# wnmusic/simpleFE

Hardware: AMD Instinct MI355X
Metric: complex-float32 MS/s through 256-tap blkconv FIR; % of HBM roofline (higher is better)
Workload: dtype f32

## Files before the change

### simplefe_amd/build.py

```python
import glob
import json
import os
import subprocess
import sys

HERE = os.path.dirname(os.path.abspath(__file__))
CSRC = os.path.join(HERE, "csrc")
LIB = os.path.join(HERE, "libsfe_dsp.so")
LIB_DIAG = os.path.join(HERE, "libsfe_dsp_diag.so")
ARCH = "gfx950"
EXACT_SOURCES = ("polyphase.hip", "util.hip", "chan.hip", "combine.hip", "ddc.hip", "psd.hip", "corr.hip", "iir.hip", "beam.hip",
                 "cov.hip", "mvdr.hip", "eig.hip", "burst.hip", "vit.hip", "mod.hip")
TICKET_SOURCES = ("fir_fft.hip", "poly_fft.hip")
HOST_SOURCES = ("api.hip", "api_plans.hip", "api_fir.hip", "api_rs.hip", "api_pipe.hip", "api_chan.hip", "api_combine.hip", "api_ddc.hip",
                "api_psd.hip", "api_corr.hip", "api_iir.hip", "api_beam.hip", "api_cov.hip", "api_mvdr.hip", "api_eig.hip", "api_burst.hip", "api_vit.hip", "api_mod.hip", "group.hip", "host.h", "block.h",
                "beam_view.h", "vit_code.h")


def sources(diag=False):
    return sorted(glob.glob(os.path.join(CSRC, "*.hip"))) + (sorted(glob.glob(os.path.join(CSRC, "diag", "*.hip"))) if diag else [])


def _deps():
    return sources(diag=True) + glob.glob(os.path.join(CSRC, "*.h")) + glob.glob(os.path.join(CSRC, "diag", "*.inc")) + glob.glob(
        os.path.join(os.path.dirname(HERE), "include", "*.h"))


KERNEL_FILES = {"fir": ("fir_fft.hip", "fft16.h", "common.h"), "resample": ("poly_fft.hip", "fft16.h", "common.h"),
                "decimate": ("polyphase.hip", "common.h"), "chan": ("chan.hip", "fft16.h", "common.h"),
                "combine": ("combine.hip", "fft16.h", "common.h"), "ddc": ("ddc.hip", "common.h"),
                "psd": ("psd.hip", "fft16.h", "common.h"), "corr": ("corr.hip", "fft16.h", "common.h"),
                "iir": ("iir.hip", "iir.h", "common.h"), "beam": ("beam.hip", "beam.h", "common.h"),
                "cov": ("cov.hip", "cov.h", "common.h"), "mvdr": ("mvdr.hip", "mvdr.h", "beam.h", "common.h"),
                "eig": ("eig.hip", "eig.h", "common.h"), "burst": ("burst.hip", "burst.h", "eig.h", "common.h"),
                "vit": ("vit.hip", "vit.h", "burst.h", "eig.h", "common.h"),
                "mod": ("mod.hip", "mod.h", "vit.h", "burst.h", "eig.h", "common.h")}


def csrc_hash(kind=None):
    import hashlib
    import re
    h = hashlib.sha256()
    paths = sorted(glob.glob(os.path.join(CSRC, "*.hip")) + glob.glob(os.path.join(CSRC, "*.h")))
    if kind is not None:
        paths = [p for p in paths if os.path.basename(p) in KERNEL_FILES[kind]]
    for p in paths:
        if os.path.basename(p) in HOST_SOURCES:
            continue
        h.update(os.path.basename(p).encode() + b"\0")
        depth, skip_at = 0, None
        for line in open(p, errors="replace"):
            code = re.sub(r"\s+", " ", re.sub(r"//.*$", "", line)).strip()
            if code.startswith("#if"):
                depth += 1
                if skip_at is None and re.match(r"#ifdef SFE_DIAG\b", code):
                    skip_at = depth
                    continue
            elif code.startswith("#else") and skip_at == depth:
                skip_at = -depth
                continue
            elif code.startswith("#endif"):
# ... 139 lines not shown
```

### simplefe_amd/csrc/api_fir.hip

```cpp
#include "host.h"

namespace sfe {


Fir *as_fir(void *h) { return as_handle<Fir>(h, "FIR"); }

static int fir_build_tables(const Fir *f, const float *taps, int parts, int ovl, FirTables &t)
{
    const int N = FFT_N;
    std::vector<double> c(N / 2), sn(N / 2);
    for (int m = 0; m < N / 2; m++) {
        c[m] = cos(-2.0 * M_PI * m / N);
        sn[m] = sin(-2.0 * M_PI * m / N);
    }
    auto fft = [&](std::vector<double> &re, std::vector<double> &im) {
        for (int i = 1, j = 0; i < N; i++) {
            int bit = N >> 1;
            for (; j & bit; bit >>= 1) j ^= bit;
            j ^= bit;
            if (i < j) {
                std::swap(re[i], re[j]);
                std::swap(im[i], im[j]);
            }
        }
// ... 15 lines not shown
    std::vector<v2f> hs((size_t)n_sets * parts * 16 * 256), tw1(7 * 256), tw2(7 * 16);
    std::vector<double> hr(N), hi(N);
    for (int set = 0; set < n_sets; set++) {
    const float *tp = taps + (size_t)set * f->n_taps * (f->taps_complex ? 2 : 1);
    for (int p = 0; p < parts; p++) {
        const int first = parts == 1 ? 0 : p * ovl;
        const int count = parts == 1 ? f->n_taps : (f->n_taps - first < ovl ? f->n_taps - first : ovl);
        for (int n = 0; n < N; n++) {
            hr[n] = n < count ? (f->taps_complex ? tp[2 * (first + n)] : tp[first + n]) / (double)N : 0.0;
            hi[n] = n < count && f->taps_complex ? tp[2 * (first + n) + 1] / (double)N : 0.0;
        }
        fft(hr, hi);
        for (int t = 0; t < 256; t++)
            for (int k0 = 0; k0 < 16; k0++) {
                const int bin = (t >> 4) + 16 * (t & 15) + 256 * k0;
                hs[(((size_t)set * parts + p) * 16 + k0) * 256 + t] = (v2f){(float)hr[bin], (float)hi[bin]};
            }
    }
    }
    for (int k = 1; k < 4; k++)
        for (int t = 0; t < 256; t++) {
            const double a = -2.0 * M_PI * (double)(t * k) / 4096.0;
            tw1[k * 256 + t] = (v2f){(float)cos(a), (float)sin(a)};
            tw1[(k + 3) * 256 + t] = (v2f){(float)cos(4.0 * a), (float)sin(4.0 * a)};
        }
    for (int k = 1; k < 4; k++)
        for (int n0 = 0; n0 < 16; n0++) {
            const double a = -2.0 * M_PI * (double)(n0 * k) / 256.0;
            tw2[k * 16 + n0] = (v2f){(float)cos(a), (float)sin(a)};
            tw2[(k + 3) * 16 + n0] = (v2f){(float)cos(4.0 * a), (float)sin(4.0 * a)};
        }
    int rc;
    if ((rc = t.hs.upload(hs)) != SFE_OK || (rc = t.tw1.upload(tw1)) != SFE_OK || (rc = t.tw2.upload(tw2)) != SFE_OK) return rc;
    return t.ticket.alloc_zero(FIR_TICKET_GROUPS_MAX * 128 / sizeof(unsigned));
}

constexpr int FIR_MAX_PARTS = 1024;
static bool fir_choose_partition(int n_taps, int *ovl, int *parts)
{
    const int need = n_taps > 1 ? n_taps - 1 : 1;
    double best = 1e300;
    *parts = 0;
    const int hl1 = ((need + 255) / 256) * 256;
    if (hl1 < FFT_N) {
        best = 1.0 / (FFT_N - hl1);
        *ovl = hl1;
        *parts = 1;
    }
    for (int o = 256; o < FFT_N; o += 256) {
        const int P = (n_taps + o - 1) / o;
        if (P < 2 || P > FIR_MAX_PARTS) continue;
        const double cost = (P + 0.25 * (P - 1)) / (FFT_N - o);
        if (cost < best) {
            best = cost;
            *ovl = o;
            *parts = P;
        }
    }
    return *parts > 0;
}

bool stream_is_capturing(hipStream_t s)
{
    hipStreamCaptureStatus cap = hipStreamCaptureStatusNone;
    if (hipStreamIsCapturing(s, &cap) != hipSuccess) {
        (void)hipGetLastError();
        return false;
// ... 73 lines not shown
        if (v == 0) best_ms = med * FIR_CAL_MARGIN;
        else if (med < best_ms) {
            best_ms = med;
            best = v;
        }
    }
    f->cal_runs++;
    {
        std::lock_guard<std::mutex> lk(g_fir_var_mutex);
        g_fir_var_cache[fir_var_key(f, a)] = best;
    }
    *chosen = best;
    return SFE_OK;
}

static void fir_fill_args(const Fir *f, FirFftArgs &a, const void *d_in, void *d_out, size_t n, size_t in_stride,
                          size_t out_stride)
{
    a.in = d_in;
    a.out = d_out;
    a.hist = f->hist.cur();
    a.tw1 = f->tab.tw1;
    a.tw2 = f->tab.tw2;
    a.n = (long long)n;
    a.in_stride = (long long)in_stride;
    a.out_stride = (long long)out_stride;
    a.hl = f->ovl;
    a.advance = FFT_N - f->ovl;
    a.hist_len = f->hl;
    a.nblk = ((long long)n + a.advance - 1) / a.advance;
    a.ticket = f->tab.ticket;
    a.total = 0;
    a.tgroups = 0;
    a.hs_stride = f->per_channel ? (long long)f->parts * 16 * 256 : 0;
    a.variant = FIR_VAR_AUTO;
    a.hs = f->tab.hs;
    a.shift = 0;
    a.hist_out = nullptr;
}

static int fir_carry_state(Fir *f, const void *d_in, size_t n, size_t in_stride, bool fused, bool capturing, hipStream_t s)
{
    const int width = f->data_complex ? 2 : 1;
    if (capturing) {
        f->captured = true;
        return launch_history_update(d_in, (long long)n, (long long)in_stride, f->hist.cur(), f->hist.cur(), f->hl,
                                     width, f->n_channels, s, f->in_u8);
    }
    if (!fused) {
        int rc = launch_history_update(d_in, (long long)n, (long long)in_stride, f->hist.cur(), f->hist.next(),
                                       f->hl, width, f->n_channels, s, f->in_u8);
        if (rc != SFE_OK) return rc;
    }
    return f->hist.carry(f->captured, s);
}

int fir_run(Fir *f, const void *d_in, void *d_out, size_t n, size_t in_stride,
                   size_t out_stride, hipStream_t s)
{
    if (n == 0) return SFE_OK;
    f->started = true;
    int algo = f->algo;
    if (algo == SFE_FIR_ALGO_AUTO) algo = f->fft_ok ? SFE_FIR_ALGO_FFT : SFE_FIR_ALGO_DIRECT;
    int rc;
    bool hist_fused = false;
    const bool capturing = stream_is_capturing(s);
// ... 416 lines not shown
    int best = FIR_VAR_REG;
    int rc = fir_calibrate(f, a, s, &best);
    if (rc == SFE_OK && chosen) *chosen = best;
    return rc;
}

int sfe_dsp_fir_forget_calibrations(void)
{
    std::lock_guard<std::mutex> lk(g_fir_var_mutex);
    g_fir_var_cache.clear();
    return SFE_OK;
}

int sfe_dsp_fir_set_zero_copy_max(sfe_fir_t h, size_t max_samples)
{
    Fir *f = as_fir(h);
    if (!f) return SFE_EINVAL;
    if (f->stage.h) {
        set_error("fir_set_zero_copy_max: set it before the first sfe_dsp_fir_process_host call");
        return SFE_ESTATE;
    }
    f->zc_max = max_samples;
    return SFE_OK;
}

int sfe_dsp_fir_reset(sfe_fir_t h)
{
    Fir *f = as_fir(h);
    if (!f) return SFE_EINVAL;
    SFE_ON_DEVICE(f->device);
    SFE_HIP(hipDeviceSynchronize());
    const int rc = f->hist.zero();
    if (rc != SFE_OK) return rc;
    if (f->tab.ticket) SFE_HIP(hipMemset(f->tab.ticket, 0, FIR_TICKET_GROUPS_MAX * 128));
    f->started = false;
    return SFE_OK;
}

int sfe_dsp_fir_destroy(sfe_fir_t h)
{
    Fir *f = as_fir(h);
    if (!f) return SFE_OK;
    if (f->piped) {
        set_error("fir_destroy: a pipe still borrows this handle (sfe_dsp_pipe_destroy first)");
        return SFE_ESTATE;
    }
    return destroy_handle(f);
}

}
```

### simplefe_amd/csrc/common.h

```cpp
#pragma once
#include <hip/hip_runtime.h>
#include <stddef.h>
#include <stdint.h>

#include "../../include/sfe_dsp.h"

typedef float v2f __attribute__((ext_vector_type(2)));
typedef float v4f __attribute__((ext_vector_type(4)));

namespace sfe {

__device__ __forceinline__ void lds_barrier()
{
#if defined(__HIP_DEVICE_COMPILE__)
    asm volatile("s_waitcnt lgkmcnt(0)" ::: "memory");
    __builtin_amdgcn_s_barrier();
    asm volatile("" ::: "memory");
#endif
}

void set_error(const char *fmt, ...);
int hip_fail(hipError_t e, const char *what);
int device_cu_count();

// ... 13 lines not shown
};

#define SFE_HIP(call)                                         \
    do {                                                      \
        hipError_t e__ = (call);                              \
        if (e__ != hipSuccess) return ::sfe::hip_fail(e__, #call); \
    } while (0)

constexpr int FFT_N = 4096;
constexpr int FFT_ROWS = 16;
constexpr int LDS_K2_STRIDE = 272;
constexpr int LDS_K1_STRIDE = 17;
constexpr int WP_PITCH = 144;
constexpr int WP_REGION = 8 * WP_PITCH;

struct FirFftArgs {
    const void *in;
    void       *out;
    const void *hist;
    void       *hist_out;
    const v2f  *hs;
    const v2f  *tw1;
    const v2f  *tw2;
    long long   n;
    long long   in_stride, out_stride;
    int         hl;
    int         advance;
    int         hist_len;
    int         shift;
    long long   nblk;
    unsigned   *ticket;
    unsigned    total;
    unsigned    tgroups;
    unsigned    ch_groups;
    long long   hs_stride;
    unsigned    tqs;
    unsigned    halo_keep;
    int         variant;
};
enum { FIR_VAR_AUTO = -1, FIR_VAR_REG = 0, FIR_VAR_DMA = 1, FIR_VAR_WP = 2, FIR_VAR_COUNT = 3 };
bool fir_fft_has_variants(const FirFftArgs &a, int in_complex, int out_complex, int in_u8, int out_tx10, int n_channels, int accumulate);
constexpr int FIR_TICKET_GROUPS = 8;
constexpr int FIR_TICKET_GROUPS_MAX = 64;
int launch_fir_fft(const FirFftArgs &a, int in_complex, int out_complex, int in_u8, int out_tx10, int n_channels,
                   hipStream_t s, int accumulate = 0);

struct PolyArgs {
    const void *in;
    void       *out;
    const void *hist;
    const float *taps;
    long long   n_in, in_stride, out_stride;
    int         hl;
    int         U, plen;
    long long   pos0;
    int         step;
    long long   n_out;
    const long long *sched_pos;
    const float     *sched_mu;
};
int launch_poly_int(const PolyArgs &a, int data_complex, int taps_complex, int exact,
                    int n_channels, hipStream_t s);

struct PolyTiledPlan {
    int    SP = 0, UP = 0, Lp = 0, e_max = 0;
    float *d_G = nullptr;
    float *d_Gt = nullptr;
    int    gt_pitch = 8;
};
struct PolyTiledArgs {
    const void *in;
    void       *out;
    const void *hist;
    void       *hist_out = nullptr;
    unsigned    tiles = 0;
    unsigned    win = 0;
// ... 117 lines not shown
```

### simplefe_amd/csrc/diag/fir_fft_diag.inc

```
template <int WAVES>
__global__ __launch_bounds__(256, WAVES) void fir_copy_pattern_kernel(FirFftArgs a)
{
    const unsigned t = threadIdx.x;
    const char *in_c = static_cast<const char *>(a.in) + (size_t)blockIdx.y * a.in_stride * 8;
    char *out_c = static_cast<char *>(a.out) + (size_t)blockIdx.y * a.out_stride * 8;
    const int row0 = a.hl >> 8;
    for (long long blk = blockIdx.x; blk < a.nblk; blk += gridDim.x) {
        const long long base = blk * a.advance - a.hl;
        if (base < 0 || base + FFT_N > a.n) continue;
        v2f v[16];
#pragma unroll
        for (int r = 0; r < 16; r++) v[r] = load_sample<true>(in_c + (base + 256 * r) * 8, t);
#pragma unroll
        for (int r = 0; r < 16; r++)
            if (r >= row0) reinterpret_cast<v2f *>(out_c + (base + 256 * r) * 8)[t] = v[r];
    }
}


template <int WAVES>
__global__ __launch_bounds__(256, WAVES) void fir_copy_pattern16_kernel(FirFftArgs a)
{
    const unsigned t = threadIdx.x;
    const char *in_c = static_cast<const char *>(a.in) + (size_t)blockIdx.y * a.in_stride * 8;
    char *out_c = static_cast<char *>(a.out) + (size_t)blockIdx.y * a.out_stride * 8;
    const int row0 = a.hl >> 8;
    const unsigned half = t >> 7, col2 = t & 127;
    for (long long blk = blockIdx.x; blk < a.nblk; blk += gridDim.x) {
        const long long base = blk * a.advance - a.hl;
        if (base < 0 || base + FFT_N > a.n) continue;
        v4f v[8];
#pragma unroll
        for (int j = 0; j < 8; j++)
            v[j] = reinterpret_cast<const v4f *>(in_c + (base + 256 * (2 * j)) * 8)[col2 + 128 * half];
#pragma unroll
        for (int j = 0; j < 8; j++)
            if (2 * j + (int)half >= row0)
                reinterpret_cast<v4f *>(out_c + (base + 256 * (2 * j)) * 8)[col2 + 128 * half] = v[j];
    }
}

#define FIR_TRACE_WGS 163840
__device__ unsigned long long g_fir_trace[5 * FIR_TRACE_WGS];
__device__ unsigned long long g_fir_tdone[FIR_TRACE_WGS];
__device__ unsigned long long g_fir_tclk[FIR_TRACE_WGS];
__device__ int g_fir_gate;
__device__ int g_fir_order;

template <int WAVES, bool TICKET, bool BAR = false, bool TRACE = false>
__global__ __launch_bounds__(256, WAVES) void fir_copy_pattern_nt_kernel(FirFftArgs a)
{
    __shared__ unsigned s_next;
    const unsigned t = threadIdx.x;
    const unsigned long long t_start = TRACE ? wall_clock64() : 0ull;
    const int gate = TRACE ? g_fir_gate : 0;
    const int order = TRACE ? g_fir_order : 0;
    unsigned n_done = 0;
    const unsigned wg_lin = blockIdx.x + blockIdx.y * gridDim.x;
    auto leave = [&]() {
        if (TRACE && t == 0 && wg_lin < FIR_TRACE_WGS) {
            unsigned long long *r = g_fir_trace + 5ull * wg_lin;
            r[0] = t_start; r[1] = wall_clock64(); r[2] = n_done;
            r[3] = __builtin_amdgcn_s_getreg(20 | (3 << 11));
            r[4] = __builtin_amdgcn_s_getreg(4 | (31 << 11));
        }
    };
    const int row0 = a.hl >> 8;
    const unsigned nblk32 = (unsigned)a.nblk;
    const unsigned tg = a.tgroups, grp = blockIdx.x % tg;
    unsigned *const my_ticket = a.ticket + 32u * grp;
    const unsigned last_draw = (a.total > grp ? (a.total - grp + tg - 1u) / tg : 0u) + (gridDim.x - grp + tg - 1u) / tg - 1u;
    auto draw = [&]() -> unsigned {
        const unsigned c = __hip_atomic_fetch_add(my_ticket, 1u, __ATOMIC_RELAXED, __HIP_MEMORY_SCOPE_AGENT);
        if (c == last_draw) __hip_atomic_store(my_ticket, 0u, __ATOMIC_RELAXED, __HIP_MEMORY_SCOPE_AGENT);
        const unsigned long long k = (unsigned long long)c * tg + grp;
        return k < a.total ? (unsigned)k : 0xFFFFFFFFu;
// ... 203 lines not shown
```

### simplefe_amd/csrc/diag/fir_fft_launch_diag.inc

```
    if (ev && in_complex && out_complex && !in_u8 && !out_tx10) {
#define SFE_NEW(DM, DG, WPV) SFE_K(true, true, false, false, false, DM, DG, false, WPV)
#define SFE_NEW_DG(DM, WPV) do { if (diag == 1) SFE_NEW(DM, 1, WPV); else if (diag == 2) SFE_NEW(DM, 2, WPV); \
                                else if (diag == 3) SFE_NEW(DM, 3, WPV); else SFE_NEW(DM, 0, WPV); } while (0)
        bool done = true;
        const bool traced = (ev[0] == 'e' || ev[0] == 'E') && (getenv("SFE_FIR_TRACE") || getenv("SFE_FIR_ORDER") || getenv("SFE_FIR_GATE"));
        if (traced) {
            const int order = getenv("SFE_FIR_ORDER") ? atoi(getenv("SFE_FIR_ORDER")) : 0;
            SFE_HIP(hipMemcpyToSymbolAsync(HIP_SYMBOL(g_fir_order), &order, sizeof order, 0, hipMemcpyHostToDevice, s));
            const int gate = getenv("SFE_FIR_GATE") ? atoi(getenv("SFE_FIR_GATE")) : 0;
            SFE_HIP(hipMemcpyToSymbolAsync(HIP_SYMBOL(g_fir_gate), &gate, sizeof gate, 0, hipMemcpyHostToDevice, s));
        }
        if (ev[0] == 'c') hipLaunchKernelGGL((fir_copy_pattern_kernel<4>), grid2, block, 0, s, a);
        else if (ev[0] == 'd') hipLaunchKernelGGL((fir_copy_pattern16_kernel<4>), grid2, block, 0, s, a);
        else if (ev[0] == 'e' && traced) hipLaunchKernelGGL((fir_copy_pattern_nt_kernel<4, false, false, true>), grid2, block, 0, s, a);
        else if (ev[0] == 'E' && traced) hipLaunchKernelGGL((fir_copy_pattern_nt_kernel<4, true, false, true>), grid, block, 0, s, a);
        else if (ev[0] == 'e') hipLaunchKernelGGL((fir_copy_pattern_nt_kernel<4, false>), grid2, block, 0, s, a);
        else if (ev[0] == 'E') hipLaunchKernelGGL((fir_copy_pattern_nt_kernel<4, true>), grid, block, 0, s, a);
        else if (ev[0] == 'b') hipLaunchKernelGGL((fir_copy_pattern_nt_kernel<4, false, true>), grid2, block, 0, s, a);
        else if (ev[0] == 'g') hipLaunchKernelGGL((fir_copy_pattern_dma_kernel<4, true>), grid2, block, 0, s, a);
        else if (ev[0] == 'G') hipLaunchKernelGGL((fir_copy_pattern_dma_kernel<4, false>), grid2, block, 0, s, a);
        else if (ev[0] == 'q' || ev[0] == 'Q') {
            const int delay = getenv("SFE_FIR_DELAY") ? atoi(getenv("SFE_FIR_DELAY")) : 0;
            SFE_HIP(hipMemcpyToSymbolAsync(HIP_SYMBOL(g_fir_delay), &delay, sizeof delay, 0, hipMemcpyHostToDevice, s));
            if (ev[0] == 'q') hipLaunchKernelGGL((fir_copy_pattern_dma2_kernel<2, true>), grid2, block, 0, s, a);
            else hipLaunchKernelGGL((fir_copy_pattern_dma2_kernel<4, false>), grid2, block, 0, s, a);
        }
        else if (ev[0] == 'p') hipLaunchKernelGGL((fir_copy_pattern_pipe_kernel<4>), grid2, block, 0, s, a);
        else if (ev[0] == 'T') SFE_NEW_DG(false, false);
        else if (ev[0] == 'X') SFE_NEW_DG(true, false);
        else if (ev[0] == 'W') SFE_NEW_DG(true, true);
        else if (ev[0] == 'y') SFE_NEW(true, 8, false);
        else if (ev[0] == 'u') SFE_NEW(false, 8, false);
        else if (ev[0] == 'L') SFE_NEW(false, 16, false);
        else if (ev[0] == 'M') SFE_NEW(false, 32, false);
        else if (ev[0] == 'N') SFE_NEW(false, 48, false);
        else if (ev[0] == 'l') SFE_NEW(true, 16, false);
        else if (ev[0] == 'n') SFE_NEW(true, 48, false);
        else if (ev[0] == 'x') SFE_NEW(true, 4, false);
        else if (ev[0] == 't') SFE_NEW(false, 4, false);
        else if (ev[0] == 'w') SFE_NEW(true, 4, true);
        else done = false;
#undef SFE_NEW
#undef SFE_NEW_DG
        if (done) {
            SFE_HIP(hipGetLastError());
            if (const char *tp = getenv("SFE_FIR_TRACE")) {
                if (traced) {
                    const size_t nwg = (ev[0] == 'E' ? (size_t)grid.x : (size_t)grid2.x * grid2.y);
                    const size_t cnt = 5 * (nwg < FIR_TRACE_WGS ? nwg : FIR_TRACE_WGS);
                    unsigned long long *h = (unsigned long long *)malloc(cnt * 8);
                    SFE_HIP(hipStreamSynchronize(s));
                    SFE_HIP(hipMemcpyFromSymbol(h, HIP_SYMBOL(g_fir_trace), cnt * 8));
                    if (FILE *f = fopen(tp, "wb")) { fwrite(h, 8, cnt, f); fclose(f); }
                    free(h);
                    const size_t nt = a.total < FIR_TRACE_WGS ? a.total : FIR_TRACE_WGS;
                    h = (unsigned long long *)malloc(nt * 8);
                    SFE_HIP(hipMemcpyFromSymbol(h, HIP_SYMBOL(g_fir_tdone), nt * 8));
                    char tp2[512];
                    snprintf(tp2, sizeof tp2, "%s.done", tp);
                    if (FILE *f = fopen(tp2, "wb")) { fwrite(h, 8, nt, f); fclose(f); }
                    SFE_HIP(hipMemcpyFromSymbol(h, HIP_SYMBOL(g_fir_tclk), nt * 8));
                    snprintf(tp2, sizeof tp2, "%s.clk", tp);
                    if (FILE *f = fopen(tp2, "wb")) { fwrite(h, 8, nt, f); fclose(f); }
                    free(h);
                }
            }
            return SFE_OK;
        }
    }
```

### simplefe_amd/csrc/fir_fft.hip

```cpp
#include <stdint.h>
#include <stdlib.h>

#include "common.h"
#include "fft16.h"

namespace sfe {
namespace {

template <bool IN_C, bool IN_U8 = false>
__device__ __forceinline__ v2f load_sample(const void *p, unsigned lane)
{
    if constexpr (IN_U8) {
        if constexpr (IN_C) {
            const unsigned w = __builtin_nontemporal_load(reinterpret_cast<const unsigned short *>(p) + lane);
            return (v2f){u8_to_f32(w & 0xFFu), u8_to_f32(w >> 8)};
        } else {
            return (v2f){u8_to_f32(__builtin_nontemporal_load(reinterpret_cast<const unsigned char *>(p) + lane)), 0.0f};
        }
    }
    if constexpr (IN_C) return __builtin_nontemporal_load(reinterpret_cast<const v2f *>(p) + lane);
    else return (v2f){__builtin_nontemporal_load(reinterpret_cast<const float *>(p) + lane), 0.0f};
}

template <int K>
__device__ __forceinline__ unsigned quad_lane(unsigned v)
{
    return (unsigned)__builtin_amdgcn_update_dpp(0, (int)v, K | (K << 2) | (K << 4) | (K << 6), 0xF, 0xF, true);
}
__device__ __forceinline__ unsigned quad_odd(unsigned v)
{
    return (unsigned)__builtin_amdgcn_update_dpp(0, (int)v, 1 | (1 << 2) | (3 << 4) | (3 << 6), 0xF, 0xF, true);
}

__device__ __forceinline__ void store_group(unsigned char *d, unsigned u0, unsigned u1, unsigned u2, unsigned u3)
{
    const unsigned w = ((u0 >> 8) | ((u1 >> 8) << 2) | ((u2 >> 8) << 4) | ((u3 >> 8) << 6)) | ((u0 & 0xFFu) << 8) |
                       ((u1 & 0xFFu) << 16) | ((u2 & 0xFFu) << 24);
    __builtin_memcpy(d, &w, 4);
    d[4] = (unsigned char)u3;
}

#ifdef SFE_DIAG
__device__ unsigned long long g_fir_clk[4];
#define SFE_FIR_STAMP(i)                                                                   \
    do {                                                                                   \
        if (blockIdx.x == 0 && blockIdx.y == 0 && threadIdx.x == 0) {                      \
            g_fir_clk[i] = __builtin_amdgcn_s_memtime();                                   \
            g_fir_clk[(i) + 1] = __builtin_amdgcn_s_memrealtime();                         \
        }                                                                                  \
    } while (0)
#else
#define SFE_FIR_STAMP(i) do { } while (0)
#endif

template <bool IN_C, bool OUT_C, bool IN_U8 = false, bool PAIR = false, bool OUT_TX10 = false, bool DMA = false, int DIAG = 0,
          bool ACC = false, bool WP = false, bool HCH = false>
__global__ __launch_bounds__(256, 4) void fir_fft4096_kernel(FirFftArgs a)
{
    static_assert(!WP || DMA, "the wave-private layout exists for the LDS-DMA path");
    static_assert(!ACC || (!OUT_TX10 && !DMA), "accumulating launches write float32 through the plain store path");
    static_assert(!DMA || (IN_C && !IN_U8 && !PAIR), "LDS-DMA input: complex float32, padded layout");
    constexpr bool INTERLEAVE = (DIAG & 8) != 0;
    constexpr bool NOMID = (DIAG & 16) != 0, NORECON = (DIAG & 32) != 0;
    auto tw2f = [](v2f x, v2f q, v2f p) -> v2f { return NORECON ? cmul(x, q) : cmul2(x, q, p); };
    auto tw2i = [](v2f x, v2f q, v2f p) -> v2f { return NORECON ? cmul_conj(x, q) : cmul2_conj(x, q, p); };
    __shared__ v2f lds[WP ? 4 * WP_REGION : FFT_ROWS * LDS_K2_STRIDE];
    __shared__ unsigned s_next;
    const unsigned t = threadIdx.x;
    SFE_FIR_STAMP(0);
    int ch = 0;
    const unsigned lo = t & 15, hi = t >> 4;
    const unsigned base_a = WP ? (t >> 6) * WP_REGION + (t & 63u) : t;
    const unsigned base_b = hi * LDS_K2_STRIDE + lo;
    const unsigned base_c = hi * LDS_K2_STRIDE + lo * LDS_K1_STRIDE;
    const unsigned base_w = (hi & 7u) * WP_PITCH + (hi >> 3) * 64u + lo;
    auto row_a = [](int r) -> unsigned { return WP ? (unsigned)((r & 7) * WP_PITCH + (r >> 3) * 64) : (unsigned)(r * LDS_K2_STRIDE); };
    auto cell_b1 = [&](int a1) -> unsigned {
        if (WP) return base_w + (unsigned)((a1 >> 2) * WP_REGION + 16 * (a1 & 3));
        return base_b + 16u * a1;
    };
    auto cell_b2 = [&](int a1) -> unsigned { return base_b + (unsigned)LDS_K1_STRIDE * a1; };
    auto cell_c = [&](int n0) -> unsigned { return base_c + n0; };

// ... 9 lines not shown
                hreg[k] = (a.hs + (size_t)c * a.hs_stride + k * 256)[threadIdx.x];
                asm volatile("" : "+v"(hreg[k]));
            }
        }
    };
    auto set_channel = [&](int c) {
        in_c = in_of(c);
        out_c = static_cast<char *>(a.out) + (OUT_TX10 ? (size_t)c * (a.out_stride * (OUT_C ? 2 : 1) / 4) * 5 : (size_t)c * a.out_stride * (OUT_C ? 8 : 4));
        hist_c = static_cast<const char *>(a.hist) + (size_t)c * a.hist_len * (IN_C ? 8 : 4);
    };
    load_spectrum(ch);
    set_channel(ch);

    v2f p1[4], q1[4], p2[4], q2[4];
#pragma unroll
    for (int k = 1; k < 4; k++) {
        p1[k] = a.tw1[k * 256 + t];
        q1[k] = a.tw1[(k + 3) * 256 + t];
        p2[k] = a.tw2[k * 16 + lo];
        q2[k] = a.tw2[(k + 3) * 16 + lo];
    }

    const int row0 = a.hl >> 8;
    auto carry_history = [&]() {
        char *ho = static_cast<char *>(a.hist_out) + (size_t)ch * a.hist_len * (IN_C ? 8 : 4);
        for (int r = 0; r < (a.hist_len >> 8); r++) {
            const v2f s = load_sample<IN_C, IN_U8>(in_c + (a.n - a.hist_len + 256 * r) * ISZ, t);
            if constexpr (IN_C) reinterpret_cast<v2f *>(ho)[256 * r + t] = s;
            else reinterpret_cast<float *>(ho)[256 * r + t] = s.x;
        }
    };
    const unsigned tg = a.tgroups, grp = blockIdx.x % tg;
    unsigned *const my_ticket = a.ticket + 32u * grp;
    const unsigned Q = 1u << a.tqs, row = tg << a.tqs, rem = a.total % row;
    const bool by_channel = HCH && a.ch_groups;
    const unsigned mine = by_channel ? (a.total / (unsigned)a.nblk / tg) * (unsigned)a.nblk
                                     : (a.total / row << a.tqs) + (rem > grp * Q ? (rem - grp * Q < Q ? rem - grp * Q : Q) : 0u);
    const unsigned last_draw = mine + (gridDim.x - grp + tg - 1u) / tg - 1u;
    const bool few = a.total <= gridDim.x;
    auto draw_issue = [&]() -> unsigned {
        if (few) return 0u;
        return __hip_atomic_fetch_add(my_ticket, 1u, __ATOMIC_RELAXED, __HIP_MEMORY_SCOPE_AGENT);
    };
    auto draw_finish = [&](unsigned c) -> unsigned {
        if (few) return 0xFFFFFFFFu;
        if (c == last_draw) __hip_atomic_store(my_ticket, 0u, __ATOMIC_RELAXED, __HIP_MEMORY_SCOPE_AGENT);
        if (by_channel) {
            if (c >= mine) return 0xFFFFFFFFu;
            const unsigned i = c / (unsigned)a.nblk;
            return (grp + tg * i) * (unsigned)a.nblk + (c - i * (unsigned)a.nblk);
        }
        const unsigned long long k = (((unsigned long long)(c >> a.tqs) * tg + grp) << a.tqs) + (c & (Q - 1u));
        return k < a.total ? (unsigned)k : 0xFFFFFFFFu;
    };
    auto draw = [&]() -> unsigned { return draw_finish(draw_issue()); };
    const unsigned nblk32 = (unsigned)a.nblk;
    if (!HCH) {
#pragma unroll
        for (int k = 0; k < 16; k++) {
            hreg[k] = (a.hs + k * 256)[t];
            asm volatile("" : "+v"(hreg[k]));
        }
    }

    auto load_rows = [&](v2f (&x)[16], long long blk) {
        constexpr int ESZ = IN_C ? 8 : 4;
        if constexpr (PAIR) {
            const long long baseA = 2 * blk * a.advance - a.hl - a.shift, baseB = baseA + a.advance;
            if constexpr (IN_U8) {
                if (baseA >= 0 && baseB + FFT_N <= a.n && (reinterpret_cast<uintptr_t>(in_c) & 15u) == 0) {
                    typedef unsigned v4u __attribute__((ext_vector_type(4)));
                    const v4u rA = __builtin_nontemporal_load(reinterpret_cast<const v4u *>(in_c + baseA) + t);
                    const v4u rB = __builtin_nontemporal_load(reinterpret_cast<const v4u *>(in_c + baseB) + t);
                    v4u *raw = reinterpret_cast<v4u *>(lds);
                    raw[t] = rA;
                    raw[256u + t] = rB;
                    lds_barrier();
                    const unsigned char *rs = reinterpret_cast<const unsigned char *>(lds);
#pragma unroll
                    for (int r = 0; r < 16; r++) x[r] = (v2f){u8_to_f32(rs[256 * r + t]), u8_to_f32(rs[4096 + 256 * r + t])};
                    lds_barrier();
                    return;
                }
            }
            if (baseA >= 0 && baseB + FFT_N <= a.n) {
#pragma unroll
                for (int r = 0; r < 16; r++)
                    x[r] = (v2f){load_sample<false, IN_U8>(in_c + (baseA + 256 * r) * ISZ, t).x,
// ... 70 lines not shown
    };
    auto dma_rows = [&](const char *chan, long long blk) {
        const char *g = chan + (blk * a.advance - a.hl - a.shift) * 8;
#pragma unroll
        for (int p = 0; p < 8; p++) {
            unsigned dst, off;
            const char *gp;
            if constexpr (WP) {
                dst = lds_base + (wv * WP_REGION + (unsigned)p * WP_PITCH) * 8u;
                gp = g + ((unsigned)p * 256u + 64u * wv) * 8u;
                off = lane_wp;
            } else {
                const unsigned row = 4u * wv + (p >> 1), half = p & 1;
                dst = lds_base + (row * LDS_K2_STRIDE + half * 128u) * 8u;
                gp = g + (row * 256u + half * 128u) * 8u;
                off = lane16;
            }
            unsigned keep;
            const bool shared_row = WP ? (((a.halo_keep >> (unsigned)p) | (a.halo_keep >> (unsigned)(p + 8))) & 1u) != 0
                                       : ((a.halo_keep >> (4u * wv + (unsigned)(p >> 1))) & 1u) != 0;
            if (shared_row)
                asm volatile("s_mov_b32 %0, m0\n\ts_mov_b32 m0, %3\n\ts_nop 0\n\tglobal_load_lds_dwordx4 %1, %2\n\ts_mov_b32 m0, %0"
                             : "=&s"(keep) : "v"(off), "s"(gp), "s"(dst) : "memory");
            else
                asm volatile("s_mov_b32 %0, m0\n\ts_mov_b32 m0, %3\n\ts_nop 0\n\tglobal_load_lds_dwordx4 %1, %2 nt\n\ts_mov_b32 m0, %0"
                             : "=&s"(keep) : "v"(off), "s"(gp), "s"(dst) : "memory");
        }
    };

    v2f nx[16];
    long long blk;
    unsigned kt_next = 0;
    {
        if (t == 0) s_next = few ? blockIdx.x : draw();
        lds_barrier();
        const unsigned kt = __builtin_amdgcn_readfirstlane(s_next);
        if (kt >= a.total) return;
        ch = (int)(kt / nblk32);
        blk = kt - (unsigned)ch * nblk32;
        load_spectrum(ch);
        set_channel(ch);
    }
    bool landed = false;
    bool counted = false;
    if (DMA && interior(blk)) {
        dma_rows(in_c, blk);
        landed = true;
    }
    for (;;) {
        v2f v[16];
        if (a.hist_out && blk == 0) carry_history();
        if (DMA && landed) {
            if (counted) asm volatile("s_waitcnt vmcnt(15)" ::: "memory");
            else asm volatile("s_waitcnt vmcnt(0)" ::: "memory");
            if (!WP) lds_barrier();
#pragma unroll
            for (int r = 0; r < 16; r++) nx[r] = lds[base_a + row_a(r)];
        } else load_rows(nx, blk);
        dft16<-1>(nx);
#pragma unroll
        for (int k = 0; k < 16; k++) {
            v2f x = nx[P16(k)];
            if ((k >> 2) && (k & 3)) x = tw2f(x, q1[k >> 2], p1[k & 3]);
            else if (k >> 2) x = cmul(x, q1[k >> 2]);
            else if (k & 3) x = cmul(x, p1[k & 3]);
            lds[base_a + row_a(k)] = x;
        }
        lds_barrier();
        unsigned drawn = 0;
// ... 2 lines not shown
        for (int r = 0; r < 16; r++) v[r] = lds[cell_b1(r)];
        dft16<-1>(v);
        if (!NOMID) lds_barrier();
        v2f wmid[16];
#pragma unroll
        for (int k = 0; k < 16; k++) {
            v2f x = v[P16(k)];
            if ((k >> 2) && (k & 3)) x = tw2f(x, q2[k >> 2], p2[k & 3]);
            else if (k >> 2) x = cmul(x, q2[k >> 2]);
            else if (k & 3) x = cmul(x, p2[k & 3]);
            if constexpr (NOMID) wmid[k] = x;
            else lds[cell_b2(k)] = x;
        }
        if (!NOMID) lds_barrier();
#pragma unroll
        for (int r = 0; r < 16; r++) {
            if constexpr (NOMID) v[r] = wmid[r];
            else v[r] = lds[cell_c(r)];
        }
        dft16<-1>(v);
        {
#pragma unroll
            for (int k = 0; k < 16; k++) v[P16(k)] = cmul(v[P16(k)], hreg[k]);
            dft16_rev<+1>(v);
#pragma unroll
            for (int k = 0; k < 16; k++) {
                if constexpr (NOMID) wmid[k] = v[k];
                else lds[cell_c(k)] = v[k];
            }
        }
        asm volatile("" : "+v"(drawn));
        if (t == 0) s_next = draw_finish(drawn);
        lds_barrier();
        kt_next = __builtin_amdgcn_readfirstlane(s_next);
        const bool more = kt_next < a.total;
        const int nch = (int)(kt_next / nblk32);
        const long long nb = kt_next - (unsigned)nch * nblk32;
        if (HCH && more && nch != ch) load_spectrum(nch);
#pragma unroll
        for (int r = 0; r < 16; r++) {
            v2f x;
            if constexpr (NOMID) x = wmid[r];
            else x = lds[cell_b2(r)];
            if ((r >> 2) && (r & 3)) x = tw2i(x, q2[r >> 2], p2[r & 3]);
            else if (r >> 2) x = cmul_conj(x, q2[r >> 2]);
            else if (r & 3) x = cmul_conj(x, p2[r & 3]);
            v[r] = x;
        }
        dft16<+1>(v);
        if (!NOMID) lds_barrier();
#pragma unroll
        for (int k = 0; k < 16; k++) lds[cell_b1(k)] = v[P16(k)];
        lds_barrier();
#pragma unroll
        for (int r = 0; r < 16; r++) {
            v2f x = lds[base_a + row_a(r)];
            if ((r >> 2) && (r & 3)) x = tw2i(x, q1[r >> 2], p1[r & 3]);
            else if (r >> 2) x = cmul_conj(x, q1[r >> 2]);
            else if (r & 3) x = cmul_conj(x, p1[r & 3]);
            v[r] = x;
        }
        if constexpr (DMA) {
            if (WP) asm volatile("s_waitcnt lgkmcnt(0)" ::: "memory");
            else lds_barrier();
            landed = more && interior(nb);
            if (landed) dma_rows(in_of(nch), nb);
            counted = landed && !OUT_TX10 && row0 == 1 && blk * a.advance + a.advance <= a.n;
// ... 129 lines not shown
            if constexpr (OUT_TX10 && OUT_C) {
                if (r < row0) continue;
                const v2f y = v[P16(r)];
                const unsigned u0 = (unsigned)((int)(short)(int)(y.x * 511.0f) + 512) & 0x3FFu;
                const unsigned u1 = (unsigned)((int)(short)(int)(y.y * 511.0f) + 512) & 0x3FFu;
                const unsigned u2 = quad_odd(u0), u3 = quad_odd(u1);
                if ((t & 1u) == 0 && orow + (long long)t + 1 < a.n) {
                    unsigned char *d = reinterpret_cast<unsigned char *>(out_c) + ((orow + (long long)t) >> 1) * 5;
                    store_group(d, u0, u1, u2, u3);
                }
                continue;
            }
            if constexpr (DIAG & 2) continue;
            if (r >= row0 && (whole || orow + (long long)t < a.n)) {
                v2f y = v[P16(r)];
                char *rp = DMA ? obase_p + (voff + (unsigned)(256 * r * OSZ)) : out_c + orow * OSZ + (size_t)t * OSZ;
                if constexpr (OUT_C) {
                    if constexpr (ACC) y += *reinterpret_cast<const v2f *>(rp);
                    __builtin_nontemporal_store(y, reinterpret_cast<v2f *>(rp));
                } else {
                    if constexpr (ACC) y.x += *reinterpret_cast<const float *>(rp);
                    __builtin_nontemporal_store(y.x, reinterpret_cast<float *>(rp));
                }
            }
        }
        }
        if constexpr (DIAG & 2) {
            v2f acc = v[0];
#pragma unroll
            for (int r = 1; r < 16; r++) acc += v[r];
            if (acc.x == 1.2345e38f) reinterpret_cast<v2f *>(out_c)[t] = acc;
        }
        }
        if (!more) break;
        blk = nb;
        if (nch != ch) {
            ch = nch;
            set_channel(ch);
        }
    }
    SFE_FIR_STAMP(2);
}


#ifdef SFE_DIAG
#include "diag/fir_fft_diag.inc"
#endif

}

#ifdef SFE_DIAG
extern "C" int sfe_dsp_diag_fir_clock(double *mhz, double *ms)
{
    unsigned long long c[4];
    SFE_HIP(hipMemcpyFromSymbol(c, HIP_SYMBOL(g_fir_clk), sizeof c));
    const double dr = (double)(c[3] - c[1]);
    if (mhz) *mhz = dr > 0 ? (double)(c[2] - c[0]) / dr * 100.0 : 0.0;
    if (ms) *ms = dr / 1e5;
    return SFE_OK;
}
#endif

bool fir_fft_has_variants(const FirFftArgs &a, int in_complex, int out_complex, int in_u8, int out_tx10, int n_channels, int accumulate)
{
    const bool dma_ok = (reinterpret_cast<uintptr_t>(a.in) & 15u) == 0 && (n_channels == 1 || (a.in_stride & 1) == 0);
    return in_complex && out_complex && !in_u8 && !out_tx10 && !accumulate && dma_ok;
}

int launch_fir_fft(const FirFftArgs &a0, int in_complex, int out_complex, int in_u8, int out_tx10, int n_channels,
                   hipStream_t s, int accumulate)
{
    FirFftArgs a = a0;
    if (a.nblk <= 0) return SFE_OK;
    if (a.hist_len < a.hl + a.shift || (a.hist_len & 255) || (a.shift & 255) || ((accumulate || a.shift) && out_tx10)) {
        set_error("fir_fft: bad partition arguments (hist_len=%d hl=%d shift=%d)", a.hist_len, a.hl, a.shift);
        return SFE_EINVAL;
    }
    if (a.hl <= 0 || (a.hl & 255) || a.hl >= FFT_N || a.advance != FFT_N - a.hl) {
        set_error("fir_fft: bad overlap rows (hl=%d advance=%d)", a.hl, a.advance);
        return SFE_EINVAL;
    }
    if (in_complex && !out_complex) {
        set_error("fir_fft: complex input with real output is not a defined combination");
        return SFE_EINVAL;
    }
    if ((out_tx10 || in_u8) && in_complex != out_complex) {
        set_error("fir_fft: wire-format input/output is built for real->real and complex->complex streams");
        return SFE_EINVAL;
    }
    int wg_per_cu = 8;
    const bool pair = !in_complex && !out_complex;
    const bool dma_ok = (reinterpret_cast<uintptr_t>(a.in) & 15u) == 0 && (n_channels == 1 || (a.in_stride & 1) == 0);
    const int var = !dma_ok ? FIR_VAR_REG : (a.variant == FIR_VAR_DMA || a.variant == FIR_VAR_WP ? a.variant : FIR_VAR_REG);
#ifdef SFE_DIAG
    const char *ev = getenv("SFE_FIR_VARIANT");
    const int diag = getenv("SFE_FIR_DIAG") ? atoi(getenv("SFE_FIR_DIAG")) & 3 : 0;
    if (const char *e = getenv("SFE_FIR_WG_PER_CU")) wg_per_cu = atoi(e) > 0 ? atoi(e) : wg_per_cu;
#endif
    long long nb = pair ? (a.nblk + 1) / 2 : a.nblk;
    a.nblk = nb;
    const long long total = nb * n_channels;
    const int cus = device_cu_count();
    long long gt = total < (long long)cus * wg_per_cu ? total : (long long)cus * wg_per_cu;
    if (total + gt >= 0xFFFFFFFFLL || !a.ticket) {
        set_error("fir_fft: %lld transforms in one launch exceed the ticket counter", total);
        return SFE_ERANGE;
    }
    a.total = (unsigned)total;
    a.tgroups = FIR_TICKET_GROUPS;
#ifdef SFE_DIAG
    if (const char *e = getenv("SFE_FIR_TGROUPS")) a.tgroups = atoi(e) >= 1 && atoi(e) <= FIR_TICKET_GROUPS_MAX ? atoi(e) : a.tgroups;
#endif
    if ((long long)a.tgroups > gt) a.tgroups = (unsigned)gt;
    a.ch_groups = a.hs_stride != 0 && a.tgroups == FIR_TICKET_GROUPS && n_channels >= (int)a.tgroups && n_channels % (int)a.tgroups == 0;
#ifdef SFE_DIAG
    if (const char *e = getenv("SFE_FIR_CH_GROUPS")) a.ch_groups = a.ch_groups && atoi(e) != 0;
#endif
    a.tqs = 3;
    a.halo_keep = 0x8001u;
#ifdef SFE_DIAG
    if (const char *e = getenv("SFE_FIR_HALO_KEEP")) a.halo_keep = (unsigned)strtoul(e, nullptr, 0);
    if (const char *e = getenv("SFE_FIR_TQS")) a.tqs = atoi(e) >= 0 && atoi(e) <= 8 ? (unsigned)atoi(e) : 0u;
#endif
    const dim3 grid((unsigned)gt), block(256);
#define SFE_K(...) hipLaunchKernelGGL((fir_fft4096_kernel<__VA_ARGS__>), grid, block, 0, s, a)
#ifdef SFE_DIAG
    long long gx = nb;
    const long long cap = ((long long)cus * wg_per_cu + n_channels - 1) / n_channels;
    if (gx > cap) gx = cap < 1 ? 1 : cap;
    const dim3 grid2((unsigned)gx, (unsigned)n_channels);
#include "diag/fir_fft_launch_diag.inc"
#endif
    if (a.hs_stride) {
        if (!in_complex || !out_complex || in_u8 || out_tx10) {
            set_error("fir_fft: per-channel taps are built for complex float32 streams");
            return SFE_EINVAL;
        }
        if (accumulate) SFE_K(true, true, false, false, false, false, 0, true, false, true);
        else if (var != FIR_VAR_REG) SFE_K(true, true, false, false, false, true, 0, false, false, true);
        else SFE_K(true, true, false, false, false, false, 0, false, false, true);
    } else if (accumulate) {
        if (in_complex) {
            if (in_u8) SFE_K(true, true, true, false, false, false, 0, true);
            else SFE_K(true, true, false, false, false, false, 0, true);
        } else if (out_complex) {
            SFE_K(false, true, false, false, false, false, 0, true);
// ... 26 lines not shown
```

Before: 336,700.

## Add cross-group work stealing to FIR ticket scheduler and halve workgroups per CU

Replaces the fixed per-group ticket dealing with a shared helper and lets a workgroup whose own ticket group is exhausted steal transforms from the group with the most remaining work. Counter reset moves from a last-draw store to a bucketed exit counter run by the final departing workgroup. The launch also drops from 8 to 4 workgroups per CU, relying on stealing to balance the tail. This adds extra atomics and peek loads at the end of each workgroup's work, and the smaller grid may reduce latency hiding.

Result: no change. 337,200 (median of 2 runs) (+0.1%).

```diff
diff --git a/simplefe_amd/build.py b/simplefe_amd/build.py
--- a/simplefe_amd/build.py
+++ b/simplefe_amd/build.py
@@ -26,7 +26,7 @@
         os.path.join(os.path.dirname(HERE), "include", "*.h"))
 
 
-KERNEL_FILES = {"fir": ("fir_fft.hip", "fft16.h", "common.h"), "resample": ("poly_fft.hip", "fft16.h", "common.h"),
+KERNEL_FILES = {"fir": ("fir_fft.hip", "fir_tickets.h", "fft16.h", "common.h"), "resample": ("poly_fft.hip", "fft16.h", "common.h"),
                 "decimate": ("polyphase.hip", "common.h"), "chan": ("chan.hip", "fft16.h", "common.h"),
                 "combine": ("combine.hip", "fft16.h", "common.h"), "ddc": ("ddc.hip", "common.h"),
                 "psd": ("psd.hip", "fft16.h", "common.h"), "corr": ("corr.hip", "fft16.h", "common.h"),
diff --git a/simplefe_amd/csrc/api_fir.hip b/simplefe_amd/csrc/api_fir.hip
--- a/simplefe_amd/csrc/api_fir.hip
+++ b/simplefe_amd/csrc/api_fir.hip
@@ -71,7 +71,7 @@
         }
     int rc;
     if ((rc = t.hs.upload(hs)) != SFE_OK || (rc = t.tw1.upload(tw1)) != SFE_OK || (rc = t.tw2.upload(tw2)) != SFE_OK) return rc;
-    return t.ticket.alloc_zero(FIR_TICKET_GROUPS_MAX * 128 / sizeof(unsigned));
+    return t.ticket.alloc_zero(FIR_TICKET_WORDS);
 }
 
 constexpr int FIR_MAX_PARTS = 1024;
@@ -211,6 +211,7 @@
     a.ticket = f->tab.ticket;
     a.total = 0;
     a.tgroups = 0;
+    a.steal = 0;
     a.hs_stride = f->per_channel ? (long long)f->parts * 16 * 256 : 0;
     a.variant = FIR_VAR_AUTO;
     a.hs = f->tab.hs;
@@ -693,7 +694,7 @@
     SFE_HIP(hipDeviceSynchronize());
     const int rc = f->hist.zero();
     if (rc != SFE_OK) return rc;
-    if (f->tab.ticket) SFE_HIP(hipMemset(f->tab.ticket, 0, FIR_TICKET_GROUPS_MAX * 128));
+    if (f->tab.ticket) SFE_HIP(hipMemset(f->tab.ticket, 0, FIR_TICKET_WORDS * sizeof(unsigned)));
     f->started = false;
     return SFE_OK;
 }
diff --git a/simplefe_amd/csrc/common.h b/simplefe_amd/csrc/common.h
--- a/simplefe_amd/csrc/common.h
+++ b/simplefe_amd/csrc/common.h
@@ -69,6 +69,7 @@
     unsigned   *ticket;
     unsigned    total;
     unsigned    tgroups;
+    unsigned    steal;
     unsigned    ch_groups;
     long long   hs_stride;
     unsigned    tqs;
@@ -79,6 +80,7 @@
 bool fir_fft_has_variants(const FirFftArgs &a, int in_complex, int out_complex, int in_u8, int out_tx10, int n_channels, int accumulate);
 constexpr int FIR_TICKET_GROUPS = 8;
 constexpr int FIR_TICKET_GROUPS_MAX = 64;
+constexpr int FIR_TICKET_WORDS = (FIR_TICKET_GROUPS_MAX + 1 + 64) * 32;
 int launch_fir_fft(const FirFftArgs &a, int in_complex, int out_complex, int in_u8, int out_tx10, int n_channels,
                    hipStream_t s, int accumulate = 0);
 
diff --git a/simplefe_amd/csrc/diag/fir_fft_diag.inc b/simplefe_amd/csrc/diag/fir_fft_diag.inc
--- a/simplefe_amd/csrc/diag/fir_fft_diag.inc
+++ b/simplefe_amd/csrc/diag/fir_fft_diag.inc
@@ -40,8 +40,6 @@
     }
 }
 
-#define FIR_TRACE_WGS 163840
-__device__ unsigned long long g_fir_trace[5 * FIR_TRACE_WGS];
 __device__ unsigned long long g_fir_tdone[FIR_TRACE_WGS];
 __device__ unsigned long long g_fir_tclk[FIR_TRACE_WGS];
 __device__ int g_fir_gate;
diff --git a/simplefe_amd/csrc/diag/fir_fft_launch_diag.inc b/simplefe_amd/csrc/diag/fir_fft_launch_diag.inc
--- a/simplefe_amd/csrc/diag/fir_fft_launch_diag.inc
+++ b/simplefe_amd/csrc/diag/fir_fft_launch_diag.inc
@@ -4,6 +4,14 @@
                                 else if (diag == 3) SFE_NEW(DM, 3, WPV); else SFE_NEW(DM, 0, WPV); } while (0)
         bool done = true;
         const bool traced = (ev[0] == 'e' || ev[0] == 'E') && (getenv("SFE_FIR_TRACE") || getenv("SFE_FIR_ORDER") || getenv("SFE_FIR_GATE"));
+        const bool ptraced = (ev[0] == 'T' || ev[0] == 'X' || ev[0] == 'W') && getenv("SFE_FIR_TRACE") && !diag;
+        if (ptraced) {
+            const unsigned zero = 0;
+            SFE_HIP(hipMemcpyToSymbolAsync(HIP_SYMBOL(g_fir_steals), &zero, sizeof zero, 0, hipMemcpyHostToDevice, s));
+            void *tr = nullptr;
+            SFE_HIP(hipGetSymbolAddress(&tr, HIP_SYMBOL(g_fir_trace)));
+            SFE_HIP(hipMemsetAsync(tr, 0, sizeof(unsigned long long) * 5 * (grid.x < FIR_TRACE_WGS ? grid.x : FIR_TRACE_WGS), s));
+        }
         if (traced) {
             const int order = getenv("SFE_FIR_ORDER") ? atoi(getenv("SFE_FIR_ORDER")) : 0;
             SFE_HIP(hipMemcpyToSymbolAsync(HIP_SYMBOL(g_fir_order), &order, sizeof order, 0, hipMemcpyHostToDevice, s));
@@ -26,6 +34,9 @@
             else hipLaunchKernelGGL((fir_copy_pattern_dma2_kernel<4, false>), grid2, block, 0, s, a);
         }
         else if (ev[0] == 'p') hipLaunchKernelGGL((fir_copy_pattern_pipe_kernel<4>), grid2, block, 0, s, a);
+        else if (ev[0] == 'T' && ptraced) SFE_NEW(false, 64, false);
+        else if (ev[0] == 'X' && ptraced) SFE_NEW(true, 64, false);
+        else if (ev[0] == 'W' && ptraced) SFE_NEW(true, 64, true);
         else if (ev[0] == 'T') SFE_NEW_DG(false, false);
         else if (ev[0] == 'X') SFE_NEW_DG(true, false);
         else if (ev[0] == 'W') SFE_NEW_DG(true, true);
@@ -45,14 +56,24 @@
         if (done) {
             SFE_HIP(hipGetLastError());
             if (const char *tp = getenv("SFE_FIR_TRACE")) {
-                if (traced) {
-                    const size_t nwg = (ev[0] == 'E' ? (size_t)grid.x : (size_t)grid2.x * grid2.y);
+                if (traced || ptraced) {
+                    const size_t nwg = (ev[0] == 'E' || ptraced ? (size_t)grid.x : (size_t)grid2.x * grid2.y);
                     const size_t cnt = 5 * (nwg < FIR_TRACE_WGS ? nwg : FIR_TRACE_WGS);
                     unsigned long long *h = (unsigned long long *)malloc(cnt * 8);
                     SFE_HIP(hipStreamSynchronize(s));
                     SFE_HIP(hipMemcpyFromSymbol(h, HIP_SYMBOL(g_fir_trace), cnt * 8));
                     if (FILE *f = fopen(tp, "wb")) { fwrite(h, 8, cnt, f); fclose(f); }
                     free(h);
+                }
+                if (ptraced) {
+                    unsigned steals = 0;
+                    SFE_HIP(hipMemcpyFromSymbol(&steals, HIP_SYMBOL(g_fir_steals), sizeof steals));
+                    char tp2[512];
+                    snprintf(tp2, sizeof tp2, "%s.steals", tp);
+                    if (FILE *f = fopen(tp2, "wb")) { fwrite(&steals, 4, 1, f); fclose(f); }
+                }
+                if (traced) {
+                    unsigned long long *h;
                     const size_t nt = a.total < FIR_TRACE_WGS ? a.total : FIR_TRACE_WGS;
                     h = (unsigned long long *)malloc(nt * 8);
                     SFE_HIP(hipMemcpyFromSymbol(h, HIP_SYMBOL(g_fir_tdone), nt * 8));
diff --git a/simplefe_amd/csrc/fir_fft.hip b/simplefe_amd/csrc/fir_fft.hip
--- a/simplefe_amd/csrc/fir_fft.hip
+++ b/simplefe_amd/csrc/fir_fft.hip
@@ -3,6 +3,7 @@
 
 #include "common.h"
 #include "fft16.h"
+#include "fir_tickets.h"
 
 namespace sfe {
 namespace {
@@ -49,6 +50,9 @@
             g_fir_clk[(i) + 1] = __builtin_amdgcn_s_memrealtime();                         \
         }                                                                                  \
     } while (0)
+#define FIR_TRACE_WGS 163840
+__device__ unsigned long long g_fir_trace[5 * FIR_TRACE_WGS];
+__device__ unsigned g_fir_steals;
 #else
 #define SFE_FIR_STAMP(i) do { } while (0)
 #endif
@@ -124,28 +128,72 @@
     };
     const unsigned tg = a.tgroups, grp = blockIdx.x % tg;
     unsigned *const my_ticket = a.ticket + 32u * grp;
-    const unsigned Q = 1u << a.tqs, row = tg << a.tqs, rem = a.total % row;
-    const bool by_channel = HCH && a.ch_groups;
-    const unsigned mine = by_channel ? (a.total / (unsigned)a.nblk / tg) * (unsigned)a.nblk
-                                     : (a.total / row << a.tqs) + (rem > grp * Q ? (rem - grp * Q < Q ? rem - grp * Q : Q) : 0u);
-    const unsigned last_draw = mine + (gridDim.x - grp + tg - 1u) / tg - 1u;
+    const FirDeal deal = {a.total, tg, a.tqs, (unsigned)a.nblk, HCH && a.ch_groups ? 1u : 0u};
+    unsigned mine = fir_share(deal, grp);
     const bool few = a.total <= gridDim.x;
+    [[maybe_unused]] constexpr bool TRACE = (DIAG & 64) != 0;
+#ifdef SFE_DIAG
+    __shared__ unsigned s_steals;
+    const unsigned long long t_start = TRACE ? wall_clock64() : 0ull;
+    unsigned n_done = 0;
+    if (TRACE && t == 0) s_steals = 0;
+#endif
     auto draw_issue = [&]() -> unsigned {
-        if (few) return 0u;
+        if (few || !mine) return 0u;
         return __hip_atomic_fetch_add(my_ticket, 1u, __ATOMIC_RELAXED, __HIP_MEMORY_SCOPE_AGENT);
     };
+    auto steal = [&]() -> unsigned {
+        if (!a.steal) return FIR_NO_TRANSFORM;
+        for (;;) {
+            unsigned victim = 0, left = 0;
+            for (unsigned first = 0; first < tg; first += FIR_PEEK_WIDTH) {
+                unsigned cnt[FIR_PEEK_WIDTH];
+#pragma unroll
+                for (unsigned k = 0; k < FIR_PEEK_WIDTH; k++)
+                    cnt[k] = __hip_atomic_load(a.ticket + 32u * (first + k), __ATOMIC_RELAXED, __HIP_MEMORY_SCOPE_AGENT);
+#pragma unroll
+                for (unsigned k = 0; k < FIR_PEEK_WIDTH; k++) cnt[k] = __builtin_amdgcn_readfirstlane(cnt[k]);
+                fir_pick_victim(deal, first, cnt, FIR_PEEK_WIDTH, victim, left);
+            }
+            if (!left) return FIR_NO_TRANSFORM;
+            const unsigned c = __builtin_amdgcn_readfirstlane(
+                __hip_atomic_fetch_add(a.ticket + 32u * victim, 1u, __ATOMIC_RELAXED, __HIP_MEMORY_SCOPE_AGENT));
+            const unsigned k = fir_ticket_transform(deal, victim, c);
+            if (k != FIR_NO_TRANSFORM) {
+#ifdef SFE_DIAG
+                if (TRACE) s_steals++;
+#endif
+                return k;
+            }
+        }
+    };
     auto draw_finish = [&](unsigned c) -> unsigned {
-        if (few) return 0xFFFFFFFFu;
-        if (c == last_draw) __hip_atomic_store(my_ticket, 0u, __ATOMIC_RELAXED, __HIP_MEMORY_SCOPE_AGENT);
-        if (by_channel) {
-            if (c >= mine) return 0xFFFFFFFFu;
-            const unsigned i = c / (unsigned)a.nblk;
-            return (grp + tg * i) * (unsigned)a.nblk + (c - i * (unsigned)a.nblk);
-        }
-        const unsigned long long k = (((unsigned long long)(c >> a.tqs) * tg + grp) << a.tqs) + (c & (Q - 1u));
-        return k < a.total ? (unsigned)k : 0xFFFFFFFFu;
-    };
-    auto draw = [&]() -> unsigned { return draw_finish(draw_issue()); };
+        if (few) return FIR_NO_TRANSFORM;
+        if (c < mine) return fir_ticket_transform(deal, grp, c);
+        return steal() | FIR_THIEF_BIT;
+    };
+    unsigned *const exit_count = a.ticket + 32u * FIR_TICKET_GROUPS_MAX;
+    auto leave = [&]() {
+        if (few) return;
+        const unsigned nb = fir_exit_buckets(gridDim.x), b = blockIdx.x % nb;
+        unsigned *const bucket = exit_count + 32u;
+        if (__hip_atomic_fetch_add(bucket + 32u * b, 1u, __ATOMIC_RELAXED, __HIP_MEMORY_SCOPE_AGENT) != fir_exit_bucket_size(gridDim.x, b) - 1u) return;
+        if (__hip_atomic_fetch_add(exit_count, 1u, __ATOMIC_RELAXED, __HIP_MEMORY_SCOPE_AGENT) != nb - 1u) return;
+        for (unsigned g = 0; g < tg; g++) __hip_atomic_store(a.ticket + 32u * g, 0u, __ATOMIC_RELAXED, __HIP_MEMORY_SCOPE_AGENT);
+        for (unsigned k = 0; k < nb; k++) __hip_atomic_store(bucket + 32u * k, 0u, __ATOMIC_RELAXED, __HIP_MEMORY_SCOPE_AGENT);
+        __hip_atomic_store(exit_count, 0u, __ATOMIC_RELAXED, __HIP_MEMORY_SCOPE_AGENT);
+    };
+    auto trace_leave = [&]() {
+#ifdef SFE_DIAG
+        if (TRACE && t == 0 && blockIdx.x < FIR_TRACE_WGS) {
+            unsigned long long *r = g_fir_trace + 5ull * blockIdx.x;
+            r[0] = t_start; r[1] = wall_clock64(); r[2] = n_done;
+            r[3] = __builtin_amdgcn_s_getreg(20 | (3 << 11));
+            r[4] = __builtin_amdgcn_s_getreg(4 | (31 << 11));
+            if (s_steals) atomicAdd(&g_fir_steals, s_steals);
+        }
+#endif
+    };
     const unsigned nblk32 = (unsigned)a.nblk;
     if (!HCH) {
 #pragma unroll
@@ -282,9 +330,17 @@
     long long blk;
     unsigned kt_next = 0;
     {
-        if (t == 0) s_next = few ? blockIdx.x : draw();
+        if (t == 0) {
+            unsigned k0 = blockIdx.x;
+            if (!few) {
+                k0 = draw_finish(draw_issue());
+                if ((k0 & ~FIR_THIEF_BIT) == FIR_NO_TRANSFORM) leave();
+            }
+            s_next = k0;
+        }
         lds_barrier();
-        const unsigned kt = __builtin_amdgcn_readfirstlane(s_next);
+        const unsigned kt = __builtin_amdgcn_readfirstlane(s_next) & ~FIR_THIEF_BIT;
+        if (__builtin_amdgcn_readfirstlane(s_next) & FIR_THIEF_BIT) mine = 0u;
         if (kt >= a.total) return;
         ch = (int)(kt / nblk32);
         blk = kt - (unsigned)ch * nblk32;
@@ -353,7 +409,8 @@
         asm volatile("" : "+v"(drawn));
         if (t == 0) s_next = draw_finish(drawn);
         lds_barrier();
-        kt_next = __builtin_amdgcn_readfirstlane(s_next);
+        kt_next = __builtin_amdgcn_readfirstlane(s_next) & ~FIR_THIEF_BIT;
+        if (__builtin_amdgcn_readfirstlane(s_next) & FIR_THIEF_BIT) mine = 0u;
         const bool more = kt_next < a.total;
         const int nch = (int)(kt_next / nblk32);
         const long long nb = kt_next - (unsigned)nch * nblk32;
@@ -549,6 +606,9 @@
             if (acc.x == 1.2345e38f) reinterpret_cast<v2f *>(out_c)[t] = acc;
         }
         }
+#ifdef SFE_DIAG
+        n_done++;
+#endif
         if (!more) break;
         blk = nb;
         if (nch != ch) {
@@ -556,6 +616,8 @@
             set_channel(ch);
         }
     }
+    if (t == 0) leave();
+    trace_leave();
     SFE_FIR_STAMP(2);
 }
 
@@ -605,7 +667,7 @@
         set_error("fir_fft: wire-format input/output is built for real->real and complex->complex streams");
         return SFE_EINVAL;
     }
-    int wg_per_cu = 8;
+    int wg_per_cu = 4;
     const bool pair = !in_complex && !out_complex;
     const bool dma_ok = (reinterpret_cast<uintptr_t>(a.in) & 15u) == 0 && (n_channels == 1 || (a.in_stride & 1) == 0);
     const int var = !dma_ok ? FIR_VAR_REG : (a.variant == FIR_VAR_DMA || a.variant == FIR_VAR_WP ? a.variant : FIR_VAR_REG);
@@ -619,7 +681,7 @@
     const long long total = nb * n_channels;
     const int cus = device_cu_count();
     long long gt = total < (long long)cus * wg_per_cu ? total : (long long)cus * wg_per_cu;
-    if (total + gt >= 0xFFFFFFFFLL || !a.ticket) {
+    if (total + gt >= (long long)FIR_NO_TRANSFORM || !a.ticket) {
         set_error("fir_fft: %lld transforms in one launch exceed the ticket counter", total);
         return SFE_ERANGE;
     }
@@ -629,6 +691,10 @@
     if (const char *e = getenv("SFE_FIR_TGROUPS")) a.tgroups = atoi(e) >= 1 && atoi(e) <= FIR_TICKET_GROUPS_MAX ? atoi(e) : a.tgroups;
 #endif
     if ((long long)a.tgroups > gt) a.tgroups = (unsigned)gt;
+    a.steal = 1;
+#ifdef SFE_DIAG
+    if (const char *e = getenv("SFE_FIR_STEAL")) a.steal = atoi(e) != 0;
+#endif
     a.ch_groups = a.hs_stride != 0 && a.tgroups == FIR_TICKET_GROUPS && n_channels >= (int)a.tgroups && n_channels % (int)a.tgroups == 0;
 #ifdef SFE_DIAG
     if (const char *e = getenv("SFE_FIR_CH_GROUPS")) a.ch_groups = a.ch_groups && atoi(e) != 0;
diff --git a/simplefe_amd/csrc/fir_tickets.h b/simplefe_amd/csrc/fir_tickets.h
--- /dev/null
+++ b/simplefe_amd/csrc/fir_tickets.h
@@ -0,0 +1,69 @@
+#pragma once
+
+#if defined(__HIPCC__) || defined(__CUDACC__)
+#define SFE_TICKET_FN __host__ __device__ inline
+#else
+#define SFE_TICKET_FN inline
+#endif
+
+namespace sfe {
+
+constexpr unsigned FIR_NO_TRANSFORM = 0x7FFFFFFFu;
+constexpr unsigned FIR_THIEF_BIT = 0x80000000u;
+constexpr unsigned FIR_EXIT_BUCKETS = 64;
+constexpr unsigned FIR_PEEK_WIDTH = 8;
+
+struct FirDeal {
+    unsigned total;
+    unsigned tgroups;
+    unsigned tqs;
+    unsigned nblk;
+    unsigned by_channel;
+};
+
+SFE_TICKET_FN unsigned fir_share(const FirDeal &d, unsigned g)
+{
+    if (d.by_channel) return (d.total / d.nblk / d.tgroups) * d.nblk;
+    const unsigned Q = 1u << d.tqs, row = d.tgroups << d.tqs, rem = d.total % row;
+    return (d.total / row << d.tqs) + (rem > g * Q ? (rem - g * Q < Q ? rem - g * Q : Q) : 0u);
+}
+
+SFE_TICKET_FN unsigned fir_ticket_transform(const FirDeal &d, unsigned g, unsigned c)
+{
+    if (d.by_channel) {
+        if (c >= fir_share(d, g)) return FIR_NO_TRANSFORM;
+        const unsigned i = c / d.nblk;
+        return (g + d.tgroups * i) * d.nblk + (c - i * d.nblk);
+    }
+    const unsigned Q = 1u << d.tqs;
+    const unsigned long long k = (((unsigned long long)(c >> d.tqs) * d.tgroups + g) << d.tqs) + (c & (Q - 1u));
+    return k < d.total ? (unsigned)k : FIR_NO_TRANSFORM;
+}
+
+SFE_TICKET_FN unsigned fir_left(const FirDeal &d, unsigned g, unsigned counter)
+{
+    const unsigned s = fir_share(d, g);
+    return s > counter ? s - counter : 0u;
+}
+
+SFE_TICKET_FN void fir_pick_victim(const FirDeal &d, unsigned first, const unsigned *counters, unsigned n, unsigned &victim, unsigned &left)
+{
+    for (unsigned k = 0; k < n; k++) {
+        const unsigned g = first + k;
+        if (g >= d.tgroups) break;
+        const unsigned l = fir_left(d, g, counters[k]);
+        if (l > left) {
+            left = l;
+            victim = g;
+        }
+    }
+}
+
+SFE_TICKET_FN unsigned fir_exit_buckets(unsigned grid) { return grid < FIR_EXIT_BUCKETS ? grid : FIR_EXIT_BUCKETS; }
+SFE_TICKET_FN unsigned fir_exit_bucket_size(unsigned grid, unsigned b)
+{
+    const unsigned nb = fir_exit_buckets(grid);
+    return (grid - b + nb - 1u) / nb;
+}
+
+}
```
